# harshad16/odh-kubeflow

Hardware: AMD Instinct MI355X
Metric: Notebook-CR reconciles/sec + p50 pod-Ready latency at 1/2/4/8 GPU pods (higher is better)
Workload: dtype n/a

## Files before the change

odh_kubeflow_amd/native/objcore.cpp:

```cpp
#define PY_SSIZE_T_CLEAN
#include <Python.h>

#include <algorithm>
#include <cerrno>
#include <cmath>
#include <cstdio>
#include <cstdlib>
#include <cstring>
#include <string>
#include <string_view>
#include <unordered_map>
#include <utility>
#include <vector>

#include "watch_feed.hpp"

namespace {

PyObject* copy_tree(PyObject* o, int depth) {
  if (depth > 512) {
    PyErr_SetString(PyExc_RecursionError, "object tree too deep");
    return nullptr;
  }
  if (PyDict_CheckExact(o)) {
    PyObject* out = _PyDict_NewPresized(PyDict_GET_SIZE(o));
    if (!out) return nullptr;
    Py_ssize_t pos = 0;
    PyObject *k, *v;
    while (PyDict_Next(o, &pos, &k, &v)) {
      PyObject* c = copy_tree(v, depth + 1);
      if (!c || PyDict_SetItem(out, k, c) < 0) {
        Py_XDECREF(c);
        Py_DECREF(out);
        return nullptr;
      }
      Py_DECREF(c);
    }
    return out;
  }
  if (PyList_CheckExact(o) || PyTuple_CheckExact(o)) {
    const bool is_list = PyList_CheckExact(o);
    const Py_ssize_t n = is_list ? PyList_GET_SIZE(o) : PyTuple_GET_SIZE(o);
    PyObject* out = PyList_New(n);
    if (!out) return nullptr;
    for (Py_ssize_t i = 0; i < n; ++i) {
      PyObject* c = copy_tree(is_list ? PyList_GET_ITEM(o, i) : PyTuple_GET_ITEM(o, i), depth + 1);
      if (!c) {
        Py_DECREF(out);
        return nullptr;
      }
      PyList_SET_ITEM(out, i, c);
    }
    return out;
  }
  if (PyDict_Check(o)) {
    PyObject* plain = PyDict_Copy(o);
    if (!plain) return nullptr;
    PyObject* r = copy_tree(plain, depth);
    Py_DECREF(plain);
    return r;
  }
  Py_INCREF(o);
  return o;
}

bool is_empty(PyObject* v) {
  if (v == Py_None) return true;
  if (PyDict_Check(v)) {
    Py_ssize_t pos = 0;
    PyObject *k, *x;
    while (PyDict_Next(v, &pos, &k, &x))
      if (!is_empty(x)) return false;
    return true;
  }
  if (PyList_Check(v)) return PyList_GET_SIZE(v) == 0;
  return false;
}

int sem_eq(PyObject* a, PyObject* b, int depth);

int dict_eq(PyObject* a, PyObject* b, int depth) {
  Py_ssize_t pos = 0;
  PyObject *k, *va;
  while (PyDict_Next(a, &pos, &k, &va)) {
    PyObject* vb = PyDict_GetItemWithError(b, k);
    if (!vb) {
      if (PyErr_Occurred()) return -1;
      if (!is_empty(va)) return 0;
      continue;
    }
    if (is_empty(va) && is_empty(vb)) continue;
    int r = sem_eq(va, vb, depth + 1);
    if (r <= 0) return r;
  }
  pos = 0;
  PyObject* vb;
  while (PyDict_Next(b, &pos, &k, &vb)) {
// ... 29 lines not shown
      PyObject* y = PySequence_Fast_GET_ITEM(fb, i);
      if (PyDict_Check(x) && PyDict_Check(y)) r = dict_eq(x, y, depth + 1);
      else r = sem_eq(x, y, depth + 1);
    }
    Py_DECREF(fa);
    Py_DECREF(fb);
    return r;
  }
  if (PyDict_Check(a) || PyDict_Check(b) || la || lb) return 0;
  return PyObject_RichCompareBool(a, b, Py_EQ);
}

PyObject* py_deepcopy(PyObject*, PyObject* o) { return copy_tree(o, 0); }

PyObject* py_semantic_equal(PyObject*, PyObject* args) {
  PyObject *a, *b;
  if (!PyArg_ParseTuple(args, "OO", &a, &b)) return nullptr;
  int r;
  if (is_empty(a) && is_empty(b)) r = 1;
  else r = sem_eq(a, b, 0);
  if (r < 0) return nullptr;
  return PyBool_FromLong(r);
}

PyObject* py_equal_except(PyObject*, PyObject* args) {
  PyObject *a, *b, *keys;
  if (!PyArg_ParseTuple(args, "O!O!O", &PyDict_Type, &a, &PyDict_Type, &b, &keys)) return nullptr;
  static PyObject* metadata_str = PyUnicode_InternFromString("metadata");
  if (PyDict_GET_SIZE(a) != PyDict_GET_SIZE(b)) Py_RETURN_FALSE;
  Py_ssize_t pos = 0;
  PyObject *k, *va;
  while (PyDict_Next(a, &pos, &k, &va)) {
    PyObject* vb = PyDict_GetItemWithError(b, k);
    if (!vb) {
      if (PyErr_Occurred()) return nullptr;
      Py_RETURN_FALSE;
    }
    int eq;
    if (PyUnicode_Check(k) && PyUnicode_Compare(k, metadata_str) == 0 && PyDict_Check(va) && PyDict_Check(vb)) {
      eq = 1;
      for (int pass = 0; pass < 2 && eq == 1; ++pass) {
        PyObject* x = pass ? vb : va;
        PyObject* y = pass ? va : vb;
        Py_ssize_t p2 = 0;
        PyObject *mk, *mv;
        while (PyDict_Next(x, &p2, &mk, &mv)) {
          int skip = PySequence_Contains(keys, mk);
          if (skip < 0) return nullptr;
          if (skip) continue;
          PyObject* other = PyDict_GetItemWithError(y, mk);
          if (!other) {
            if (PyErr_Occurred()) return nullptr;
            eq = 0;
            break;
          }
          if (pass == 0) {
            int r = PyObject_RichCompareBool(mv, other, Py_EQ);
            if (r < 0) return nullptr;
            if (!r) {
              eq = 0;
              break;
            }
          }
        }
      }
    } else {
      eq = PyObject_RichCompareBool(va, vb, Py_EQ);
      if (eq < 0) return nullptr;
    }
    if (!eq) Py_RETURN_FALSE;
  }
  Py_RETURN_TRUE;
}



struct Parser {
  const char* p;
  const char* end;
  std::string buf;
  std::vector<PyObject*> stack;
  bool strip_mf = false;
  bool meta_next = false;
};

struct Frame {
  Parser& ps;
  size_t base;
  explicit Frame(Parser& p) : ps(p), base(p.stack.size()) {}
  ~Frame() {
    for (size_t i = base; i < ps.stack.size(); ++i) Py_XDECREF(ps.stack[i]);
    ps.stack.resize(base);
  }
  size_t size() const { return ps.stack.size() - base; }
  PyObject*& at(size_t i) { return ps.stack[base + i]; }
};

std::unordered_map<std::string_view, PyObject*>* g_keys = nullptr;
constexpr size_t kMaxKeys = 1 << 15;

inline void ws(Parser& ps) {
  while (ps.p < ps.end && (*ps.p == ' ' || *ps.p == '\n' || *ps.p == '\r' || *ps.p == '\t')) ++ps.p;
}

PyObject* fail(Parser&, const char* what) {
  if (!PyErr_Occurred()) PyErr_Format(PyExc_ValueError, "invalid JSON: %s", what);
  return nullptr;
}

void put_utf8(std::string& out, uint32_t cp) {
  if (cp < 0x80) {
    out.push_back(static_cast<char>(cp));
  } else if (cp < 0x800) {
    out.push_back(static_cast<char>(0xC0 | (cp >> 6)));
    out.push_back(static_cast<char>(0x80 | (cp & 0x3F)));
  } else if (cp < 0x10000) {
    out.push_back(static_cast<char>(0xE0 | (cp >> 12)));
    out.push_back(static_cast<char>(0x80 | ((cp >> 6) & 0x3F)));
    out.push_back(static_cast<char>(0x80 | (cp & 0x3F)));
  } else {
    out.push_back(static_cast<char>(0xF0 | (cp >> 18)));
    out.push_back(static_cast<char>(0x80 | ((cp >> 12) & 0x3F)));
    out.push_back(static_cast<char>(0x80 | ((cp >> 6) & 0x3F)));
    out.push_back(static_cast<char>(0x80 | (cp & 0x3F)));
  }
}

int hex4(const char* s, uint32_t* out) {
  uint32_t v = 0;
  for (int i = 0; i < 4; ++i) {
    char c = s[i];
    v <<= 4;
    if (c >= '0' && c <= '9') v |= c - '0';
    else if (c >= 'a' && c <= 'f') v |= c - 'a' + 10;
    else if (c >= 'A' && c <= 'F') v |= c - 'A' + 10;
    else return -1;
  }
  *out = v;
  return 0;
}

bool scan_string(Parser& ps, const char** s, Py_ssize_t* n, bool* ascii) {
  const char* start = ps.p;
  bool hi = false;
  while (ps.p < ps.end) {
    unsigned char c = static_cast<unsigned char>(*ps.p);
    if (c == '"') {
      *s = start;
      *n = ps.p - start;
      *ascii = !hi;
      ++ps.p;
      return true;
    }
    if (c == '\\') break;
    if (c >= 0x80) hi = true;
    ++ps.p;
  }
  if (ps.p >= ps.end) {
    PyErr_SetString(PyExc_ValueError, "invalid JSON: unterminated string");
    return false;
  }
  ps.buf.assign(start, ps.p - start);
  while (ps.p < ps.end) {
    unsigned char c = static_cast<unsigned char>(*ps.p);
    if (c == '"') {
      ++ps.p;
      *s = ps.buf.data();
// ... 98 lines not shown
  if (it != g_keys->end()) {
    Py_INCREF(it->second);
    return it->second;
  }
  PyObject* u = make_str(s, n, true);
  if (!u) return nullptr;
  PyUnicode_InternInPlace(&u);
  if (g_keys->size() < kMaxKeys && PyUnicode_IS_ASCII(u)) {
    Py_INCREF(u);
    g_keys->emplace(std::string_view(static_cast<const char*>(PyUnicode_DATA(u)), static_cast<size_t>(n)), u);
  }
  return u;
}

PyObject* number_value(Parser& ps, PyObject* old) {
  const char* start = ps.p;
  bool is_float = false;
  if (ps.p < ps.end && *ps.p == '-') ++ps.p;
  while (ps.p < ps.end) {
    char c = *ps.p;
    if (c >= '0' && c <= '9') {
      ++ps.p;
    } else if (c == '.' || c == 'e' || c == 'E' || c == '+' || c == '-') {
      is_float = true;
      ++ps.p;
    } else {
      break;
    }
  }
  if (ps.p == start || (ps.p - start == 1 && *start == '-')) return fail(ps, "bad number");
  if (!is_float) {
    const char* q = start;
    const bool neg = *q == '-';
    if (neg) ++q;
    if (ps.p - q <= 18 && (ps.p - q == 1 || *q != '0')) {
      long long v = 0;
      for (; q < ps.p; ++q) v = v * 10 + (*q - '0');
      if (neg) v = -v;
      if (old && PyLong_CheckExact(old)) {
        int overflow = 0;
        long long ov = PyLong_AsLongLongAndOverflow(old, &overflow);
        if (!overflow && ov == v && !PyErr_Occurred()) {
          Py_INCREF(old);
          return old;
        }
        PyErr_Clear();
      }
      return PyLong_FromLongLong(v);
    }
  }
  ps.buf.assign(start, ps.p - start);
  if (!is_float) {
    errno = 0;
    char* e = nullptr;
    long long v = std::strtoll(ps.buf.c_str(), &e, 10);
    if (errno == 0 && e && *e == '\0') {
      if (old && PyLong_CheckExact(old)) {
        int overflow = 0;
        long long ov = PyLong_AsLongLongAndOverflow(old, &overflow);
        if (!overflow && ov == v && !PyErr_Occurred()) {
          Py_INCREF(old);
          return old;
        }
        PyErr_Clear();
      }
      return PyLong_FromLongLong(v);
    }
    PyObject* big = PyLong_FromString(ps.buf.c_str(), nullptr, 10);
    return big ? same_or(big, old) : nullptr;
  }
  char* e = nullptr;
  double d = std::strtod(ps.buf.c_str(), &e);
  if (!e || *e != '\0') return fail(ps, "bad number");
  if (old && PyFloat_CheckExact(old) && PyFloat_AS_DOUBLE(old) == d) {
    Py_INCREF(old);
    return old;
  }
  return PyFloat_FromDouble(d);
}

PyObject* value(Parser& ps, PyObject* old, int depth);
bool skip_value(Parser& ps, int depth);

PyObject* object_value(Parser& ps, PyObject* old, int depth) {
  PyObject* od = (old && PyDict_CheckExact(old)) ? old : nullptr;
  Frame f(ps);
  bool same = od != nullptr;
  Py_ssize_t pos = 0;
  bool in_step = od != nullptr;
  const bool strip_here = ps.meta_next;
  ps.meta_next = false;
  ws(ps);
  if (ps.p < ps.end && *ps.p == '}') {
    ++ps.p;
  } else {
    while (true) {
      ws(ps);
      if (ps.p >= ps.end || *ps.p != '"') return fail(ps, "expected a key");
      ++ps.p;
      const char* ks;
      Py_ssize_t kn;
      bool kascii;
      if (!scan_string(ps, &ks, &kn, &kascii)) return nullptr;
      if (strip_here && kn == 13 && std::memcmp(ks, "managedFields", 13) == 0) {
        ws(ps);
        if (ps.p >= ps.end || *ps.p != ':') return fail(ps, "expected ':'");
        ++ps.p;
        if (!skip_value(ps, depth + 1)) return fail(ps, "bad managedFields");
        ws(ps);
        if (ps.p < ps.end && *ps.p == ',') {
          ++ps.p;
          continue;
        }
        if (ps.p < ps.end && *ps.p == '}') {
          ++ps.p;
          break;
        }
        return fail(ps, "expected ',' or '}'");
      }
      const bool meta = ps.strip_mf && depth == 0 && kn == 8 && std::memcmp(ks, "metadata", 8) == 0;
      PyObject* key = nullptr;
      PyObject* ov = nullptr;
      if (in_step) {
        PyObject *k2, *v2;
        if (PyDict_Next(od, &pos, &k2, &v2) && PyUnicode_CheckExact(k2) && PyUnicode_IS_ASCII(k2) && kascii &&
            PyUnicode_GET_LENGTH(k2) == kn && std::memcmp(PyUnicode_DATA(k2), ks, static_cast<size_t>(kn)) == 0) {
          key = k2;
          Py_INCREF(key);
          ov = v2;
        } else {
          in_step = false;
        }
      }
      if (!key) {
        key = key_object(ks, kn, kascii);
        if (!key) return nullptr;
        ov = od ? PyDict_GetItemWithError(od, key) : nullptr;
        if (!ov && PyErr_Occurred()) PyErr_Clear();
      }
      ps.stack.push_back(key);
      ws(ps);
      if (ps.p >= ps.end || *ps.p != ':') return fail(ps, "expected ':'");
      ++ps.p;
      ps.meta_next = meta;
      PyObject* v = value(ps, ov, depth + 1);
      ps.meta_next = false;
      if (!v) return nullptr;
      ps.stack.push_back(v);
      if (v != ov) same = false;
      ws(ps);
      if (ps.p < ps.end && *ps.p == ',') {
        ++ps.p;
        continue;
      }
      if (ps.p < ps.end && *ps.p == '}') {
        ++ps.p;
        break;
      }
      return fail(ps, "expected ',' or '}'");
    }
  }
  const Py_ssize_t n = static_cast<Py_ssize_t>(f.size() / 2);
  if (same && in_step && depth > 0 && n == PyDict_GET_SIZE(od)) {
    Py_INCREF(od);
    return od;
  }
  PyObject* out = _PyDict_NewPresized(n);
  if (!out) return nullptr;
  for (Py_ssize_t i = 0; i < n; ++i) {
    if (PyDict_SetItem(out, f.at(2 * i), f.at(2 * i + 1)) < 0) {
      Py_DECREF(out);
      return nullptr;
    }
  }
  if (same && depth > 0 && PyDict_GET_SIZE(out) == PyDict_GET_SIZE(od)) {
    Py_DECREF(out);
    Py_INCREF(od);
    return od;
  }
  return out;
}

PyObject* array_value(Parser& ps, PyObject* old, int depth) {
  PyObject* ol = (old && PyList_CheckExact(old)) ? old : nullptr;
  Frame f(ps);
  bool same = ol != nullptr;
  ws(ps);
  if (ps.p < ps.end && *ps.p == ']') {
    ++ps.p;
  } else {
    while (true) {
      Py_ssize_t i = static_cast<Py_ssize_t>(f.size());
      PyObject* ov = (ol && i < PyList_GET_SIZE(ol)) ? PyList_GET_ITEM(ol, i) : nullptr;
      PyObject* v = value(ps, ov, depth + 1);
      if (!v) return nullptr;
      ps.stack.push_back(v);
      if (v != ov) same = false;
      ws(ps);
      if (ps.p < ps.end && *ps.p == ',') {
        ++ps.p;
        continue;
      }
      if (ps.p < ps.end && *ps.p == ']') {
        ++ps.p;
        break;
      }
      return fail(ps, "expected ',' or ']'");
    }
  }
  const size_t n = f.size();
  if (same && depth > 0 && static_cast<Py_ssize_t>(n) == PyList_GET_SIZE(ol)) {
    Py_INCREF(ol);
    return ol;
  }
  PyObject* out = PyList_New(static_cast<Py_ssize_t>(n));
  if (!out) return nullptr;
  for (size_t i = 0; i < n; ++i) {
    PyList_SET_ITEM(out, static_cast<Py_ssize_t>(i), f.at(i));
    f.at(i) = nullptr;
  }
  return out;
}

bool literal(Parser& ps, const char* word, size_t n) {
  if (static_cast<size_t>(ps.end - ps.p) >= n && std::memcmp(ps.p, word, n) == 0) {
    ps.p += n;
    return true;
  }
  return false;
// ... 149 lines not shown
    ws(ps);
    if (ps.p < ps.end && *ps.p == ',') {
      ++ps.p;
      continue;
    }
    return;
  }
}

bool init_parser(PyObject* data, Parser* ps) {
  char* buf;
  Py_ssize_t n;
  if (PyBytes_Check(data)) {
    if (PyBytes_AsStringAndSize(data, &buf, &n) < 0) return false;
  } else if (PyByteArray_Check(data)) {
    buf = PyByteArray_AS_STRING(data);
    n = PyByteArray_GET_SIZE(data);
  } else if (PyUnicode_Check(data)) {
    const char* s = PyUnicode_AsUTF8AndSize(data, &n);
    if (!s) return false;
    buf = const_cast<char*>(s);
  } else {
    PyErr_SetString(PyExc_TypeError, "expected bytes or str");
    return false;
  }
  ps->p = buf;
  ps->end = buf + n;
  return true;
}

PyObject* py_loads_shared(PyObject*, PyObject* args) {
  PyObject *data, *old = Py_None;
  if (!PyArg_ParseTuple(args, "O|O", &data, &old)) return nullptr;
  Parser ps;
  if (!init_parser(data, &ps)) return nullptr;
  PyObject* out = value(ps, old == Py_None ? nullptr : old, 0);
  if (!out) return nullptr;
  ws(ps);
  if (ps.p != ps.end) {
    Py_DECREF(out);
    return fail(ps, "extra data");
  }
  return out;
}

template <class Lookup>
bool decode_event(Parser& ps, Lookup&& lookup, PyObject** type_out, PyObject** obj_out) {
  ws(ps);
  if (ps.p >= ps.end || *ps.p != '{') {
    fail(ps, "an event is an object");
    return false;
  }
  ++ps.p;
  PyObject* type = nullptr;
  PyObject* obj = nullptr;
  bool ok = false;
  ws(ps);
  if (ps.p < ps.end && *ps.p == '}') {
    ++ps.p;
  } else {
    while (true) {
      ws(ps);
      if (ps.p >= ps.end || *ps.p != '"') {
        fail(ps, "expected a key");
        goto done;
      }
      ++ps.p;
      const char* ks;
      Py_ssize_t kn;
      bool ascii;
      if (!scan_string(ps, &ks, &kn, &ascii)) goto done;
      bool is_type = kn == 4 && std::memcmp(ks, "type", 4) == 0;
      bool is_obj = kn == 6 && std::memcmp(ks, "object", 6) == 0;
      ws(ps);
      if (ps.p >= ps.end || *ps.p != ':') {
        fail(ps, "expected ':'");
        goto done;
      }
      ++ps.p;
      if (is_obj) {
        PyObject* old = nullptr;
        std::string ns, name;
        peek_key(ps, &ns, &name);
        if (!name.empty() && !lookup(ns, name, &old)) goto done;
        Py_XDECREF(obj);
        obj = value(ps, old, 0);
        Py_XDECREF(old);
        if (!obj) goto done;
      } else {
        PyObject* v = value(ps, nullptr, 1);
        if (!v) goto done;
        if (is_type) {
          Py_XDECREF(type);
          type = v;
        } else {
          Py_DECREF(v);
        }
      }
      ws(ps);
      if (ps.p < ps.end && *ps.p == ',') {
        ++ps.p;
        continue;
      }
      if (ps.p < ps.end && *ps.p == '}') {
        ++ps.p;
        break;
      }
      fail(ps, "expected ',' or '}'");
      goto done;
    }
  }
  ws(ps);
  if (ps.p != ps.end) {
    fail(ps, "extra data");
    goto done;
  }
  if (!obj) obj = PyDict_New();
  if (!obj) goto done;
  if (!type) {
    type = Py_None;
    Py_INCREF(type);
  }
  ok = true;
done:
  if (!ok) {
    Py_XDECREF(type);
    Py_XDECREF(obj);
    return false;
  }
  *type_out = type;
  *obj_out = obj;
  return true;
}

PyObject* py_loads_event(PyObject*, PyObject* args) {
  PyObject *data, *lookup = Py_None;
  if (!PyArg_ParseTuple(args, "O|O", &data, &lookup)) return nullptr;
  Parser ps;
  if (!init_parser(data, &ps)) return nullptr;
  PyObject *type, *obj;
  auto find = [lookup](const std::string& ns, const std::string& name, PyObject** old) {
    if (lookup == Py_None) return true;
    PyObject* r = PyObject_CallFunction(lookup, "s#s#", ns.data(), static_cast<Py_ssize_t>(ns.size()),
                                        name.data(), static_cast<Py_ssize_t>(name.size()));
    if (!r) return false;
    if (r != Py_None) *old = r;
    else Py_DECREF(r);
    return true;
  };
  if (!decode_event(ps, find, &type, &obj)) return nullptr;
  PyObject* ret = PyTuple_Pack(2, type, obj);
  Py_DECREF(type);
  Py_DECREF(obj);
  return ret;
}


bool enc_value(std::string& out, PyObject* o, int depth);

void enc_string(std::string& out, PyObject* u) {
  Py_ssize_t n;
  const char* s = PyUnicode_AsUTF8AndSize(u, &n);
  out.push_back('"');
  const char* run = s;
  for (Py_ssize_t i = 0; i < n; ++i) {
    unsigned char c = static_cast<unsigned char>(s[i]);
    if (c >= 0x20 && c != '"' && c != '\\') continue;
    out.append(run, static_cast<size_t>(s + i - run));
    run = s + i + 1;
// ... 136 lines not shown
      case '\\': out.append("\\\\"); break;
      case '\n': out.append("\\n"); break;
      case '\r': out.append("\\r"); break;
      case '\t': out.append("\\t"); break;
      case '\b': out.append("\\b"); break;
      case '\f': out.append("\\f"); break;
      default:
        if (c >= 0x10000) {
          const uint32_t v = c - 0x10000;
          u4(0xD800 | ((v >> 10) & 0x3FF));
          u4(0xDC00 | (v & 0x3FF));
        } else {
          u4(c);
        }
    }
  }
  out.push_back('"');
}

bool canon_value(std::string& out, PyObject* o, int depth) {
  if (depth > 512) {
    PyErr_SetString(PyExc_ValueError, "too deep");
    return false;
  }
  if (PyUnicode_CheckExact(o)) {
    canon_string(out, o);
    return true;
  }
  if (PyDict_CheckExact(o)) {
    std::vector<std::pair<PyObject*, PyObject*>> members;
    members.reserve(static_cast<size_t>(PyDict_GET_SIZE(o)));
    Py_ssize_t pos = 0;
    PyObject *k, *v;
    while (PyDict_Next(o, &pos, &k, &v)) {
      if (!PyUnicode_CheckExact(k)) {
        PyErr_SetString(PyExc_TypeError, "non-str key");
        return false;
      }
      members.emplace_back(k, v);
    }
    std::sort(members.begin(), members.end(),
              [](const auto& a, const auto& b) { return PyUnicode_Compare(a.first, b.first) < 0; });
    out.push_back('{');
    bool first = true;
    for (const auto& kv : members) {
      if (!first) out.push_back(',');
      first = false;
      canon_string(out, kv.first);
      out.push_back(':');
      if (!canon_value(out, kv.second, depth + 1)) return false;
    }
    out.push_back('}');
    return true;
  }
  if (PyList_CheckExact(o) || PyTuple_CheckExact(o)) {
    const bool list = PyList_CheckExact(o);
    const Py_ssize_t n = list ? PyList_GET_SIZE(o) : PyTuple_GET_SIZE(o);
    out.push_back('[');
    for (Py_ssize_t i = 0; i < n; ++i) {
      if (i) out.push_back(',');
      if (!canon_value(out, list ? PyList_GET_ITEM(o, i) : PyTuple_GET_ITEM(o, i), depth + 1)) return false;
    }
    out.push_back(']');
    return true;
  }
  if (PyUnicode_Check(o) || PyDict_Check(o) || PyList_Check(o)) {
    PyErr_SetString(PyExc_TypeError, "not a plain JSON tree");
    return false;
  }
  return enc_value(out, o, depth);
}

PyObject* py_canonical(PyObject*, PyObject* o) {
  std::string out;
  out.reserve(1024);
  if (!canon_value(out, o, 0)) {
    if (!PyErr_Occurred()) PyErr_SetString(PyExc_TypeError, "not a JSON tree");
    return nullptr;
  }
  return PyBytes_FromStringAndSize(out.data(), static_cast<Py_ssize_t>(out.size()));
}


struct WatchStore {
  PyObject_HEAD
  PyObject* items;
  PyObject* api_version;
  PyObject* kind;
  bool namespaced;
  watchfeed::Framer* framer;
  std::string* failed;
  Parser* ps;
};

PyObject* g_str_metadata = nullptr;
PyObject* g_str_namespace = nullptr;
PyObject* g_str_name = nullptr;
PyObject* g_str_api_version = nullptr;
PyObject* g_str_kind = nullptr;
PyObject* g_str_empty = nullptr;

void ws_dealloc(WatchStore* self) {
  Py_XDECREF(self->items);
  Py_XDECREF(self->api_version);
  Py_XDECREF(self->kind);
  delete self->framer;
  delete self->failed;
  delete self->ps;
  PyTypeObject* type = Py_TYPE(self);
  type->tp_free(reinterpret_cast<PyObject*>(self));
  Py_DECREF(type);
}

PyObject* ws_new(PyTypeObject* type, PyObject* args, PyObject* kw) {
  static const char* names[] = {"api_version", "kind", "namespaced", nullptr};
  PyObject *av, *kind;
  int namespaced = 1;
  if (!PyArg_ParseTupleAndKeywords(args, kw, "UU|p", const_cast<char**>(names), &av, &kind, &namespaced))
    return nullptr;
  WatchStore* self = reinterpret_cast<WatchStore*>(type->tp_alloc(type, 0));
  if (!self) return nullptr;
  self->framer = new watchfeed::Framer();
  self->failed = new std::string();
  self->ps = new Parser();
  self->ps->strip_mf = true;
  self->namespaced = namespaced != 0;
  Py_INCREF(av);
  self->api_version = av;
  Py_INCREF(kind);
  self->kind = kind;
  self->items = PyDict_New();
  if (!self->items) {
    Py_DECREF(self);
    return nullptr;
  }
  return reinterpret_cast<PyObject*>(self);
}

PyObject* ws_begin(WatchStore* self, PyObject* arg) {
  const long long want = PyLong_AsLongLong(arg);
  if (want == -1 && PyErr_Occurred()) return nullptr;
  try {
    self->framer->begin(want);
  } catch (const watchfeed::FrameError& e) {
    PyErr_SetString(PyExc_ValueError, e.what());
    return nullptr;
  }
  self->failed->clear();
  Py_RETURN_NONE;
}

PyObject* meta_field(PyObject* obj, PyObject* which) {
  PyObject* md = PyDict_GetItemWithError(obj, g_str_metadata);
  PyObject* v = nullptr;
  if (md && PyDict_Check(md)) v = PyDict_GetItemWithError(md, which);
  if (!v) {
    if (PyErr_Occurred()) return nullptr;
    v = g_str_empty;
  }
  Py_INCREF(v);
  return v;
}

enum LineResult { kLineOk, kLineStop, kLineFailed, kLineError };

LineResult ws_line(WatchStore* self, const char* s, size_t n, bool apply, PyObject* out) {
  Parser& ps = *self->ps;
  ps.p = s;
  ps.end = s + n;
  ps.meta_next = false;
  PyObject* type = nullptr;
  PyObject* obj = nullptr;
  auto find = [self](const std::string& ns, const std::string& name, PyObject** old) {
    PyObject* k = Py_BuildValue("(s#s#)", self->namespaced ? ns.data() : "",
                                self->namespaced ? static_cast<Py_ssize_t>(ns.size()) : Py_ssize_t{0}, name.data(),
                                static_cast<Py_ssize_t>(name.size()));
    if (!k) {
      PyErr_Clear();
      return true;
    }
    PyObject* hit = PyDict_GetItemWithError(self->items, k);
    Py_DECREF(k);
    if (!hit && PyErr_Occurred()) return false;
    Py_XINCREF(hit);
    *old = hit;
    return true;
  };
  PyObject* entry = nullptr;
  if (!decode_event(ps, find, &type, &obj)) {
    if (PyErr_ExceptionMatches(PyExc_RecursionError)) {
      PyErr_Clear();
      *self->failed = "invalid JSON: nested deeper than 512";
      return kLineFailed;
    }
    if (!PyErr_ExceptionMatches(PyExc_ValueError)) return kLineError;
    PyErr_Clear();
  } else if (!PyUnicode_CheckExact(type) || !PyDict_CheckExact(obj)) {
    Py_CLEAR(type);
    Py_CLEAR(obj);
  }
  if (!type) {
    PyObject* raw = PyBytes_FromStringAndSize(s, static_cast<Py_ssize_t>(n));
    if (!raw) return kLineError;
    entry = PyTuple_Pack(3, Py_None, raw, Py_None);
    Py_DECREF(raw);
    if (!entry || PyList_Append(out, entry) < 0) {
      Py_XDECREF(entry);
      return kLineError;
    }
    Py_DECREF(entry);
    return kLineOk;
  }
  LineResult res = kLineOk;
  PyObject* old = nullptr;
  const bool is_error = PyUnicode_CompareWithASCIIString(type, "ERROR") == 0;
  if (is_error) {
    res = kLineStop;
  } else if (PyUnicode_CompareWithASCIIString(type, "BOOKMARK") != 0) {
    if (!PyDict_SetDefault(obj, g_str_api_version, self->api_version) ||
        !PyDict_SetDefault(obj, g_str_kind, self->kind))
      res = kLineError;
    if (res == kLineOk && apply) {
      PyObject* ns = meta_field(obj, g_str_namespace);
      PyObject* name = ns ? meta_field(obj, g_str_name) : nullptr;
      PyObject* k = name ? PyTuple_Pack(2, ns, name) : nullptr;
      Py_XDECREF(ns);
      Py_XDECREF(name);
      if (!k) {
        res = kLineError;
      } else {
        old = PyDict_GetItemWithError(self->items, k);
        Py_XINCREF(old);
        if (!old && PyErr_Occurred()) {
          res = kLineError;
        } else if (PyUnicode_CompareWithASCIIString(type, "DELETED") == 0) {
          if (old && PyDict_DelItem(self->items, k) < 0) res = kLineError;
        } else if (PyDict_SetItem(self->items, k, obj) < 0) {
          res = kLineError;
        }
        Py_DECREF(k);
      }
    }
  }
  if (res != kLineError) {
    entry = PyTuple_Pack(3, type, obj, old ? old : Py_None);
    if (!entry || PyList_Append(out, entry) < 0) res = kLineError;
    Py_XDECREF(entry);
  }
  Py_XDECREF(old);
  Py_DECREF(type);
  Py_DECREF(obj);
  return res;
}

PyObject* ws_feed(WatchStore* self, PyObject* args, PyObject* kw) {
  static const char* names[] = {"data", "apply", nullptr};
  Py_buffer view;
  int apply = 1;
  if (!PyArg_ParseTupleAndKeywords(args, kw, "y*|p", const_cast<char**>(names), &view, &apply)) return nullptr;
  if (!self->failed->empty()) {
    PyBuffer_Release(&view);
    PyErr_SetString(PyExc_ValueError, self->failed->c_str());
    return nullptr;
  }
  PyObject* out = PyList_New(0);
  if (!out) {
    PyBuffer_Release(&view);
    return nullptr;
  }
  bool error = false;
  try {
    self->framer->feed(static_cast<const char*>(view.buf), static_cast<size_t>(view.len),
                       [&](const char* s, size_t n) {
                         const LineResult r = ws_line(self, s, n, apply != 0, out);
                         if (r == kLineError) error = true;
                         return r == kLineOk;
                       });
  } catch (const watchfeed::FrameError& e) {
    *self->failed = std::string("bad watch response body: ") + e.what();
  }
  PyBuffer_Release(&view);
  self->ps->p = self->ps->end = nullptr;
  if (error) {
    Py_DECREF(out);
    return nullptr;
  }
  if (!self->failed->empty() && PyList_GET_SIZE(out) == 0) {
    Py_DECREF(out);
    PyErr_SetString(PyExc_ValueError, self->failed->c_str());
    return nullptr;
  }
  return out;
}

PyObject* ws_get_items(WatchStore* self, void*) {
  Py_INCREF(self->items);
  return self->items;
}

PyObject* ws_get_done(WatchStore* self, void*) { return PyBool_FromLong(self->framer->done()); }

PyObject* ws_get_failed(WatchStore* self, void*) {
  if (self->failed->empty()) Py_RETURN_NONE;
  return PyUnicode_FromStringAndSize(self->failed->data(), static_cast<Py_ssize_t>(self->failed->size()));
}

PyMethodDef ws_methods[] = {
    {"begin", reinterpret_cast<PyCFunction>(ws_begin), METH_O,
     "begin(want): a response body starts (-2 chunked, -3 until EOF, else its Content-Length)."},
    {"feed", reinterpret_cast<PyCFunction>(reinterpret_cast<void (*)(void)>(ws_feed)), METH_VARARGS | METH_KEYWORDS,
     "feed(data, apply=True) -> [(type, new, old)]: the events these body bytes complete."},
    {nullptr, nullptr, 0, nullptr}};

PyGetSetDef ws_getset[] = {
    {"items", reinterpret_cast<getter>(ws_get_items), nullptr, "(namespace, name) -> object", nullptr},
    {"done", reinterpret_cast<getter>(ws_get_done), nullptr, "the body has ended", nullptr},
    {"failed", reinterpret_cast<getter>(ws_get_failed), nullptr, "why the body cannot be read further, or None",
     nullptr},
    {nullptr, nullptr, nullptr, nullptr, nullptr}};

PyType_Slot ws_slots[] = {
    {Py_tp_doc, const_cast<char*>("An informer's objects, fed with the bytes of its watch response.")},
    {Py_tp_new, reinterpret_cast<void*>(ws_new)},
    {Py_tp_dealloc, reinterpret_cast<void*>(ws_dealloc)},
    {Py_tp_methods, ws_methods},
    {Py_tp_getset, ws_getset},
    {0, nullptr}};

PyType_Spec ws_spec = {"_objcore.WatchStore", sizeof(WatchStore), 0, Py_TPFLAGS_DEFAULT, ws_slots};

bool init_watch_store(PyObject* m) {
  g_str_metadata = PyUnicode_InternFromString("metadata");
  g_str_namespace = PyUnicode_InternFromString("namespace");
  g_str_name = PyUnicode_InternFromString("name");
  g_str_api_version = PyUnicode_InternFromString("apiVersion");
  g_str_kind = PyUnicode_InternFromString("kind");
  g_str_empty = PyUnicode_InternFromString("");
  if (!g_str_metadata || !g_str_namespace || !g_str_name || !g_str_api_version || !g_str_kind || !g_str_empty)
    return false;
  PyObject* type = PyType_FromSpec(&ws_spec);
  if (!type) return false;
  if (PyModule_AddObject(m, "WatchStore", type) < 0) {
    Py_DECREF(type);
    return false;
  }
  return true;
}

PyMethodDef methods[] = {
    {"canonical", py_canonical, METH_O,
     "canonical(obj) -> bytes: json.dumps(obj, sort_keys=True, separators=(',', ':')) of a plain JSON tree."},
    {"dumps", py_dumps, METH_O,
     "dumps(obj) -> bytes: compact JSON (json.dumps with separators=(',', ':'), UTF-8) of a JSON tree."},
    {"deepcopy", py_deepcopy, METH_O, "Deep copy of a JSON tree (dict/list; tuples become lists)."},
    {"semantic_equal", py_semantic_equal, METH_VARARGS,
     "Structural equality treating missing/None/{}/[] map values as equal."},
    {"equal_except", py_equal_except, METH_VARARGS, "a == b ignoring the given metadata keys."},
    {"loads_shared", py_loads_shared, METH_VARARGS,
     "loads_shared(data, old=None): json.loads, reusing the subtrees of old the document leaves unchanged."},
    {"loads_event", py_loads_event, METH_VARARGS,
     "loads_event(line, lookup=None) -> (type, object): a watch event, the object decoded against "
     "lookup(namespace, name)."},
    {nullptr, nullptr, 0, nullptr}};

PyModuleDef module = {PyModuleDef_HEAD_INIT, "_objcore", "Native JSON-tree core", -1, methods,
                      nullptr, nullptr, nullptr, nullptr};

}

PyMODINIT_FUNC PyInit__objcore(void) {
  if (!g_keys) g_keys = new std::unordered_map<std::string_view, PyObject*>();
  PyObject* m = PyModule_Create(&module);
  if (m && !init_watch_store(m)) {
    Py_DECREF(m);
    return nullptr;
  }
  return m;
}
```

odh_kubeflow_amd/ops/build.py:

```python

from __future__ import annotations

import os
import shutil
import subprocess
import sys
import sysconfig
from typing import Dict, List

HERE = os.path.dirname(os.path.abspath(__file__))
CSRC = os.path.join(HERE, "csrc")
LIBDIR = os.path.join(HERE, "_lib")
NATIVE = os.path.join(os.path.dirname(HERE), "native")
TEST_NATIVE = os.path.join(os.path.dirname(HERE), "testing", "native")
OBJCORE = "_objcore" + (sysconfig.get_config_var("EXT_SUFFIX") or ".so")
ARCH = os.environ.get("ODH_GPU_ARCH", "gfx950")
ROCM = os.environ.get("ROCM_PATH", "/opt/rocm")
PROBE_EXE = "odh-gpu-probe"


def _hipcc() -> str:
    p = os.path.join(ROCM, "bin", "hipcc")
    return p if os.path.exists(p) else (shutil.which("hipcc") or p)


def targets() -> Dict[str, dict]:
    return {
        "libodh_gpu_probe.so": {
            "src": [os.path.join(CSRC, "gpu_probe.hip"), os.path.join(CSRC, "probe_cli.cpp")],
            "deps": [os.path.join(CSRC, "gpu_probe.h"), os.path.join(CSRC, "gpu_probe_mx.h"),
                     os.path.join(CSRC, "gpu_probe_dense.h"), os.path.join(CSRC, "gpu_probe_fp.h"),
                     os.path.join(CSRC, "gpu_probe_sparse.h"), os.path.join(CSRC, "gpu_probe_cvt.h"),
                     os.path.join(CSRC, "gpu_probe_lds.h")],
            "cmd": lambda src, out: [_hipcc(), f"--offload-arch={ARCH}", "-O3", "-std=c++17", "-shared", "-fPIC",
                                     *src, "-o", out],
        },
        PROBE_EXE: {
            "src": [os.path.join(CSRC, "probe_main.cpp")],
            "deps": [os.path.join(LIBDIR, "libodh_gpu_probe.so")],
            "cmd": lambda src, out: [_hipcc(), "-O2", "-std=c++17", *src, f"-L{LIBDIR}", "-lodh_gpu_probe",
                                     "-Wl,-rpath,$ORIGIN", "-o", out],
        },
        OBJCORE: {
            "src": [os.path.join(NATIVE, "objcore.cpp")],
            "deps": [os.path.join(NATIVE, "watch_feed.hpp")],
            "out": os.path.join(NATIVE, OBJCORE),
            "cmd": lambda src, out: [os.environ.get("CXX", "g++"), "-O2", "-std=c++17", "-shared", "-fPIC", "-Wall",
                                     "-fno-strict-aliasing", f"-I{sysconfig.get_paths()['include']}", *src,
                                     "-o", out],
        },
        "odh-apiserver": {
            "src": [os.path.join(TEST_NATIVE, "apiserver", "apiserver.cpp")],
            "deps": [os.path.join(TEST_NATIVE, "apiserver", "json.hpp")],
            "out": os.path.join(TEST_NATIVE, "bin", "odh-apiserver"),
            "cmd": lambda src, out: [os.environ.get("CXX", "g++"), "-O2", "-std=c++17", "-pthread", "-Wall", *src,
                                     "-o", out, "-lssl", "-lcrypto"],
        },
        "libodh_gpu_telemetry.so": {
            "src": [os.path.join(CSRC, "gpu_telemetry.cpp")],
            "cmd": lambda src, out: [os.environ.get("CXX", "g++"), "-O2", "-std=c++17", "-shared", "-fPIC",
                                     "-pthread", "-Wall", *src, "-o", out],
        },
    }


def lib_path(name: str) -> str:
    return os.path.join(LIBDIR, name)


def _stale(out: str, srcs: List[str]) -> bool:
    if not os.path.exists(out):
        return True
    t = os.path.getmtime(out)
    return any(os.path.getmtime(s) > t for s in srcs)


HOST_TARGETS = (OBJCORE, "libodh_gpu_telemetry.so")
PROBE_TARGETS = ("libodh_gpu_probe.so", PROBE_EXE)


def build(force: bool = False, verbose: bool = True, only=None) -> Dict[str, str]:
    os.makedirs(LIBDIR, exist_ok=True)
    built = {}
    for name, spec in targets().items():
        if only is not None and name not in only:
            continue
        out = spec.get("out") or lib_path(name)
        os.makedirs(os.path.dirname(out), exist_ok=True)
        if force or _stale(out, spec["src"] + spec.get("deps", [])):
            tmp = out + ".tmp"
            cmd = spec["cmd"](spec["src"], tmp)
            if verbose:
                print("[build]", " ".join(cmd), flush=True)
            subprocess.run(cmd, check=True)
            os.replace(tmp, out)
        built[name] = out
    return built


if __name__ == "__main__":
    sel = None
    if "--host-only" in sys.argv:
        sel = HOST_TARGETS
    elif "--probe-only" in sys.argv:
        sel = PROBE_TARGETS
    build(force="--force" in sys.argv, only=sel)
```

Baseline: 3861.

## Reuse unchanged JSON subtrees across watch events via recorded text spans

Records, for each stored object, the raw JSON text and a span table covering the top-level metadata, spec and status members. On the next event for the same object, a member whose bytes are identical to the previous text is skipped and the old Python value is reused, with no re-parsing. This is meant to cut parse and allocation cost when watch events repeat mostly unchanged objects. In exchange it keeps a per-object text copy in memory, and the sync pass now walks the whole cache. It is enabled by default through reuse_text.

```diff
diff --git a/odh_kubeflow_amd/native/objcore.cpp b/odh_kubeflow_amd/native/objcore.cpp
--- a/odh_kubeflow_amd/native/objcore.cpp
+++ b/odh_kubeflow_amd/native/objcore.cpp
@@ -13,6 +13,7 @@
 #include <utility>
 #include <vector>
 
+#include "span_reuse.hpp"
 #include "watch_feed.hpp"
 
 namespace {
@@ -208,7 +209,12 @@
   std::vector<PyObject*> stack;
   bool strip_mf = false;
   bool meta_next = false;
+  spanreuse::Table* rec = nullptr;
+  const spanreuse::Table* prev = nullptr;
+  const char* base = nullptr;
 };
+
+constexpr int32_t kNoSpans = -2;
 
 struct Frame {
   Parser& ps;
@@ -473,7 +479,67 @@
 PyObject* value(Parser& ps, PyObject* old, int depth);
 bool skip_value(Parser& ps, int depth);
 
+struct SpanWalk {
+  int32_t parent = kNoSpans;
+  int32_t first = -1, cur = -1;
+  int32_t last = -1;
+};
+
+template <bool kSpans>
+PyObject* object_members(Parser& ps, PyObject* old, int depth, SpanWalk walk);
+
+PyObject* spanned_value(Parser& ps, PyObject* old, int depth, int32_t parent, int32_t first) {
+  if (ps.p < ps.end && *ps.p == '{') {
+    ++ps.p;
+    SpanWalk walk;
+    walk.parent = parent;
+    walk.first = walk.cur = first;
+    return object_members<true>(ps, old, depth, walk);
+  }
+  return value(ps, old, depth);
+}
+
+__attribute__((noinline)) PyObject* spanned_member(Parser& ps, PyObject* ov, int depth, bool meta, const char* kraw,
+                                                   size_t kraw_n, SpanWalk& walk) {
+  ws(ps);
+  const int32_t span = walk.last = ps.rec->open(walk.parent, walk.last, static_cast<size_t>(kraw - ps.base), kraw_n,
+                                                static_cast<size_t>(ps.p - ps.base));
+  const bool sub = depth == 0 && ((kraw_n == 8 && std::memcmp(kraw, "metadata", 8) == 0) ||
+                                  (kraw_n == 4 && std::memcmp(kraw, "spec", 4) == 0) ||
+                                  (kraw_n == 6 && std::memcmp(kraw, "status", 6) == 0));
+  PyObject* v = nullptr;
+  int32_t child = -1;
+  const int32_t os =
+      walk.first >= 0 ? ps.prev->find(walk.first, walk.cur, ps.prev->text.data(), kraw, kraw_n) : -1;
+  if (os >= 0) {
+    const spanreuse::Span& o = ps.prev->spans[static_cast<size_t>(os)];
+    walk.cur = o.next;
+    if (ov && o.handle == ov) {
+      if (ps.prev->same(os, ps.p, ps.end)) {
+        ps.p += ps.prev->length(os);
+        ps.rec->adopt(span, *ps.prev, os);
+        Py_INCREF(ov);
+        v = ov;
+      } else {
+        child = o.child;
+      }
+    }
+  }
+  if (!v) {
+    ps.meta_next = meta;
+    v = sub ? spanned_value(ps, ov, depth + 1, span, child) : value(ps, ov, depth + 1);
+  }
+  ps.meta_next = false;
+  if (v) ps.rec->close(span, static_cast<size_t>(ps.p - ps.base), v);
+  return v;
+}
+
 PyObject* object_value(Parser& ps, PyObject* old, int depth) {
+  return object_members<false>(ps, old, depth, SpanWalk());
+}
+
+template <bool kSpans>
+PyObject* object_members(Parser& ps, PyObject* old, int depth, SpanWalk walk) {
   PyObject* od = (old && PyDict_CheckExact(old)) ? old : nullptr;
   Frame f(ps);
   bool same = od != nullptr;
@@ -489,10 +555,12 @@
       ws(ps);
       if (ps.p >= ps.end || *ps.p != '"') return fail(ps, "expected a key");
       ++ps.p;
+      [[maybe_unused]] const char* const kraw = ps.p;
       const char* ks;
       Py_ssize_t kn;
       bool kascii;
       if (!scan_string(ps, &ks, &kn, &kascii)) return nullptr;
+      [[maybe_unused]] const char* const kraw_end = ps.p - 1;
       if (strip_here && kn == 13 && std::memcmp(ks, "managedFields", 13) == 0) {
         ws(ps);
         if (ps.p >= ps.end || *ps.p != ':') return fail(ps, "expected ':'");
@@ -533,9 +601,14 @@
       ws(ps);
       if (ps.p >= ps.end || *ps.p != ':') return fail(ps, "expected ':'");
       ++ps.p;
-      ps.meta_next = meta;
-      PyObject* v = value(ps, ov, depth + 1);
-      ps.meta_next = false;
+      PyObject* v;
+      if constexpr (kSpans) {
+        v = spanned_member(ps, ov, depth, meta, kraw, static_cast<size_t>(kraw_end - kraw), walk);
+      } else {
+        ps.meta_next = meta;
+        v = value(ps, ov, depth + 1);
+        ps.meta_next = false;
+      }
       if (!v) return nullptr;
       ps.stack.push_back(v);
       if (v != ov) same = false;
@@ -851,9 +924,20 @@
         PyObject* old = nullptr;
         std::string ns, name;
         peek_key(ps, &ns, &name);
+        if (ps.rec) {
+          ps.rec->clear();
+          ps.prev = nullptr;
+        }
         if (!name.empty() && !lookup(ns, name, &old)) goto done;
         Py_XDECREF(obj);
-        obj = value(ps, old, 0);
+        if (ps.rec) {
+          ws(ps);
+          ps.base = ps.p;
+          obj = spanned_value(ps, old, 0, spanreuse::kRoot, ps.prev ? ps.prev->root : -1);
+        } else {
+          obj = value(ps, old, 0);
+        }
+        if (ps.rec && obj) ps.rec->text.assign(ps.base, static_cast<size_t>(ps.p - ps.base));
         Py_XDECREF(old);
         if (!obj) goto done;
       } else {
@@ -1156,6 +1240,12 @@
 }
 
 
+struct TextEntry {
+  PyObject* obj = nullptr;
+  size_t ns_len = 0;
+  spanreuse::Table table;
+};
+
 struct WatchStore {
   PyObject_HEAD
   PyObject* items;
@@ -1165,7 +1255,19 @@
   watchfeed::Framer* framer;
   std::string* failed;
   Parser* ps;
+  std::unordered_map<std::string, TextEntry>* texts;
+  spanreuse::Table* rec;
+  std::string* peeked;
+  size_t peeked_ns;
 };
+
+void drop_text(WatchStore* self, const std::string& key) {
+  auto it = self->texts->find(key);
+  if (it == self->texts->end()) return;
+  PyObject* obj = it->second.obj;
+  self->texts->erase(it);
+  Py_XDECREF(obj);
+}
 
 PyObject* g_str_metadata = nullptr;
 PyObject* g_str_namespace = nullptr;
@@ -1181,16 +1283,22 @@
   delete self->framer;
   delete self->failed;
   delete self->ps;
+  if (self->texts)
+    for (auto& kv : *self->texts) Py_XDECREF(kv.second.obj);
+  delete self->texts;
+  delete self->rec;
+  delete self->peeked;
   PyTypeObject* type = Py_TYPE(self);
   type->tp_free(reinterpret_cast<PyObject*>(self));
   Py_DECREF(type);
 }
 
 PyObject* ws_new(PyTypeObject* type, PyObject* args, PyObject* kw) {
-  static const char* names[] = {"api_version", "kind", "namespaced", nullptr};
+  static const char* names[] = {"api_version", "kind", "namespaced", "reuse_text", nullptr};
   PyObject *av, *kind;
-  int namespaced = 1;
-  if (!PyArg_ParseTupleAndKeywords(args, kw, "UU|p", const_cast<char**>(names), &av, &kind, &namespaced))
+  int namespaced = 1, reuse_text = 1;
+  if (!PyArg_ParseTupleAndKeywords(args, kw, "UU|pp", const_cast<char**>(names), &av, &kind, &namespaced,
+                                   &reuse_text))
     return nullptr;
   WatchStore* self = reinterpret_cast<WatchStore*>(type->tp_alloc(type, 0));
   if (!self) return nullptr;
@@ -1198,6 +1306,11 @@
   self->failed = new std::string();
   self->ps = new Parser();
   self->ps->strip_mf = true;
+  if (reuse_text) {
+    self->texts = new std::unordered_map<std::string, TextEntry>();
+    self->rec = new spanreuse::Table();
+    self->peeked = new std::string();
+  }
   self->namespaced = namespaced != 0;
   Py_INCREF(av);
   self->api_version = av;
@@ -1221,6 +1334,25 @@
     return nullptr;
   }
   self->failed->clear();
+  if (self->texts) {
+    std::vector<PyObject*> gone;
+    for (auto it = self->texts->begin(); it != self->texts->end();) {
+      const TextEntry& e = it->second;
+      const std::string& key = it->first;
+      PyObject* k = Py_BuildValue("(s#s#)", key.data(), static_cast<Py_ssize_t>(e.ns_len), key.data() + e.ns_len + 1,
+                                  static_cast<Py_ssize_t>(key.size() - e.ns_len - 1));
+      PyObject* hit = k ? PyDict_GetItemWithError(self->items, k) : nullptr;
+      Py_XDECREF(k);
+      if (PyErr_Occurred()) PyErr_Clear();
+      if (hit == e.obj) {
+        ++it;
+      } else {
+        gone.push_back(e.obj);
+        it = self->texts->erase(it);
+      }
+    }
+    for (PyObject* o : gone) Py_XDECREF(o);
+  }
   Py_RETURN_NONE;
 }
 
@@ -1243,9 +1375,17 @@
   ps.p = s;
   ps.end = s + n;
   ps.meta_next = false;
+  ps.prev = nullptr;
+  ps.rec = nullptr;
+  if (self->texts && n <= UINT32_MAX) {
+    ps.rec = self->rec;
+    ps.rec->clear();
+    self->peeked->clear();
+  }
   PyObject* type = nullptr;
   PyObject* obj = nullptr;
   auto find = [self](const std::string& ns, const std::string& name, PyObject** old) {
+    if (self->ps->rec) self->peeked->clear();
     PyObject* k = Py_BuildValue("(s#s#)", self->namespaced ? ns.data() : "",
                                 self->namespaced ? static_cast<Py_ssize_t>(ns.size()) : Py_ssize_t{0}, name.data(),
                                 static_cast<Py_ssize_t>(name.size()));
@@ -1256,14 +1396,29 @@
     PyObject* hit = PyDict_GetItemWithError(self->items, k);
     Py_DECREF(k);
     if (!hit && PyErr_Occurred()) return false;
+    if (self->ps->rec) {
+      std::string& key = *self->peeked;
+      self->peeked_ns = self->namespaced ? ns.size() : 0;
+      if (self->namespaced) key = ns;
+      key.push_back('\0');
+      key += name;
+      if (hit) {
+        auto it = self->texts->find(key);
+        if (it != self->texts->end() && it->second.obj == hit) self->ps->prev = &it->second.table;
+      }
+    }
     Py_XINCREF(hit);
     *old = hit;
     return true;
   };
   PyObject* entry = nullptr;
-  if (!decode_event(ps, find, &type, &obj)) {
+  const bool decoded = decode_event(ps, find, &type, &obj);
+  const bool undecoded =
+      ps.rec && !self->peeked->empty() && (!decoded || !PyUnicode_CheckExact(type) || !PyDict_CheckExact(obj));
+  if (!decoded) {
     if (PyErr_ExceptionMatches(PyExc_RecursionError)) {
       PyErr_Clear();
+      if (undecoded) drop_text(self, *self->peeked);
       *self->failed = "invalid JSON: nested deeper than 512";
       return kLineFailed;
     }
@@ -1273,6 +1428,7 @@
     Py_CLEAR(type);
     Py_CLEAR(obj);
   }
+  if (undecoded) drop_text(self, *self->peeked);
   if (!type) {
     PyObject* raw = PyBytes_FromStringAndSize(s, static_cast<Py_ssize_t>(n));
     if (!raw) return kLineError;
@@ -1315,6 +1471,19 @@
         Py_DECREF(k);
       }
     }
+    if (res == kLineOk && ps.rec && !self->peeked->empty()) {
+      if (PyUnicode_CompareWithASCIIString(type, "DELETED") == 0 || ps.rec->text.empty()) {
+        drop_text(self, *self->peeked);
+      } else {
+        TextEntry& e = (*self->texts)[*self->peeked];
+        PyObject* was = e.obj;
+        Py_INCREF(obj);
+        e.obj = obj;
+        e.ns_len = self->peeked_ns;
+        std::swap(e.table, *ps.rec);
+        Py_XDECREF(was);
+      }
+    }
   }
   if (res != kLineError) {
     entry = PyTuple_Pack(3, type, obj, old ? old : Py_None);
@@ -1379,6 +1548,10 @@
   return PyUnicode_FromStringAndSize(self->failed->data(), static_cast<Py_ssize_t>(self->failed->size()));
 }
 
+PyObject* ws_get_text_entries(WatchStore* self, void*) {
+  return PyLong_FromSize_t(self->texts ? self->texts->size() : 0);
+}
+
 PyMethodDef ws_methods[] = {
     {"begin", reinterpret_cast<PyCFunction>(ws_begin), METH_O,
      "begin(want): a response body starts (-2 chunked, -3 until EOF, else its Content-Length)."},
@@ -1391,6 +1564,8 @@
     {"done", reinterpret_cast<getter>(ws_get_done), nullptr, "the body has ended", nullptr},
     {"failed", reinterpret_cast<getter>(ws_get_failed), nullptr, "why the body cannot be read further, or None",
      nullptr},
+    {"text_entries", reinterpret_cast<getter>(ws_get_text_entries), nullptr,
+     "how many objects' texts are kept (reuse_text)", nullptr},
     {nullptr, nullptr, nullptr, nullptr, nullptr}};
 
 PyType_Slot ws_slots[] = {
diff --git a/odh_kubeflow_amd/native/span_reuse.hpp b/odh_kubeflow_amd/native/span_reuse.hpp
--- /dev/null
+++ b/odh_kubeflow_amd/native/span_reuse.hpp
@@ -0,0 +1,92 @@
+#pragma once
+
+#include <cstddef>
+#include <cstdint>
+#include <cstring>
+#include <string>
+#include <vector>
+
+namespace spanreuse {
+
+inline bool same_text(const char* p, const char* end, const char* old, size_t len) {
+  if (len == 0 || p > end || static_cast<size_t>(end - p) < len || std::memcmp(p, old, len) != 0) return false;
+  const char c = old[0];
+  if (c == '{' || c == '[' || c == '"') return true;
+  if (static_cast<size_t>(end - p) == len) return false;
+  const char d = p[len];
+  return d == ',' || d == '}' || d == ']' || d == ' ' || d == '\n' || d == '\r' || d == '\t';
+}
+
+struct Span {
+  uint32_t key, key_len;
+  uint32_t begin, end;
+  int32_t next;
+  int32_t child;
+  void* handle;
+};
+
+constexpr int32_t kRoot = -1;
+
+struct Table {
+  std::string text;
+  std::vector<Span> spans;
+  int32_t root = -1;
+
+  void clear() {
+    text.clear();
+    spans.clear();
+    root = -1;
+  }
+
+  int32_t open(int32_t parent, int32_t last, size_t key, size_t key_len, size_t begin) {
+    const int32_t i = static_cast<int32_t>(spans.size());
+    spans.push_back(Span{static_cast<uint32_t>(key), static_cast<uint32_t>(key_len), static_cast<uint32_t>(begin),
+                         static_cast<uint32_t>(begin), -1, -1, nullptr});
+    if (last >= 0) spans[static_cast<size_t>(last)].next = i;
+    else if (parent >= 0) spans[static_cast<size_t>(parent)].child = i;
+    else root = i;
+    return i;
+  }
+
+  void close(int32_t i, size_t end, void* handle) {
+    spans[static_cast<size_t>(i)].end = static_cast<uint32_t>(end);
+    spans[static_cast<size_t>(i)].handle = handle;
+  }
+
+  int32_t find(int32_t first, int32_t cur, const char* from, const char* k, size_t n) const {
+    if (cur < 0) cur = first;
+    for (int32_t i = cur; i >= 0; i = spans[static_cast<size_t>(i)].next)
+      if (key_is(i, from, k, n)) return i;
+    for (int32_t i = first; i >= 0 && i != cur; i = spans[static_cast<size_t>(i)].next)
+      if (key_is(i, from, k, n)) return i;
+    return -1;
+  }
+
+  bool key_is(int32_t i, const char* from, const char* k, size_t n) const {
+    const Span& s = spans[static_cast<size_t>(i)];
+    return s.key_len == n && std::memcmp(from + s.key, k, n) == 0;
+  }
+
+  bool same(int32_t i, const char* p, const char* end) const {
+    const Span& s = spans[static_cast<size_t>(i)];
+    return same_text(p, end, text.data() + s.begin, s.end - s.begin);
+  }
+
+  size_t length(int32_t i) const {
+    const Span& s = spans[static_cast<size_t>(i)];
+    return s.end - s.begin;
+  }
+
+  void adopt(int32_t to, const Table& old, int32_t from) {
+    const Span& o = old.spans[static_cast<size_t>(from)];
+    const uint32_t at = spans[static_cast<size_t>(to)].begin;
+    int32_t last = -1;
+    for (int32_t c = o.child; c >= 0; c = old.spans[static_cast<size_t>(c)].next) {
+      const Span& s = old.spans[static_cast<size_t>(c)];
+      last = open(to, last, s.key - o.begin + at, s.key_len, s.begin - o.begin + at);
+      close(last, s.end - o.begin + at, s.handle);
+    }
+  }
+};
+
+}
diff --git a/odh_kubeflow_amd/ops/build.py b/odh_kubeflow_amd/ops/build.py
--- a/odh_kubeflow_amd/ops/build.py
+++ b/odh_kubeflow_amd/ops/build.py
@@ -43,7 +43,7 @@
         },
         OBJCORE: {
             "src": [os.path.join(NATIVE, "objcore.cpp")],
-            "deps": [os.path.join(NATIVE, "watch_feed.hpp")],
+            "deps": [os.path.join(NATIVE, "watch_feed.hpp"), os.path.join(NATIVE, "span_reuse.hpp")],
             "out": os.path.join(NATIVE, OBJCORE),
             "cmd": lambda src, out: [os.environ.get("CXX", "g++"), "-O2", "-std=c++17", "-shared", "-fPIC", "-Wall",
                                      "-fno-strict-aliasing", f"-I{sysconfig.get_paths()['include']}", *src,
```

Measured after the change: 3856 (median of 2 runs). No clear change (-0.1%).
